# muditbhargava66/FFT-implementation-in-C

Measured on AMD Instinct MI355X. Metric: Gpoint/s + achieved HBM GB/s, batched 1D c2c FFT at 1/2/4/8 MI355X, higher is better.
Workload: dtype f32; 1 GPU; N=1048576 fp32 complex, batch=512 per GPU (BASELINE configs[2], north-star); n=1048576, batch_per_gpu=512, batch_total=512, direction=forward, placement=out-of-place, parallelism=batch index sharded over 1 GPU(s), one process per GPU, no collectives, algo=auto, passes=2, chunk_batch=128, bluestein_m=0, schedule=team kernel: one HBM round trip, a whole transform per team of CUs of one XCD, team_tiles=4, team_status=0, device=AMD Radeon Graphics (gfx950:sramecc+:xnack-, 256 CUs)

## Files before the change

fft-implementation-in-c_amd/csrc/fft_device.h:

```cpp
#pragma once

#include <stdint.h>

#if defined(FFT_EMU)
#include <cstring>
namespace emu {
struct dim3_ { unsigned x, y, z; };
extern thread_local dim3_ threadIdx_;
extern thread_local dim3_ blockIdx_;
extern dim3_ blockDim_;
extern dim3_ gridDim_;
extern thread_local unsigned char* smem_;
void sync_threads();
long long clock_ticks();
extern int xcc_skew;
unsigned shfl_xor_u32(unsigned v, int mask);
}
#define FFT_KERNEL
#define FFT_DEVICE inline
#define FFT_HOST_DEVICE inline
#define FFT_TID ((int)emu::threadIdx_.x)
#define FFT_BID ((long long)emu::blockIdx_.x)
#define FFT_NTHREADS ((int)emu::blockDim_.x)
#define FFT_NBLOCKS ((long long)emu::gridDim_.x)
// ... 9 lines not shown
    memcpy(w, &v, sizeof(T));
    for (unsigned i = 0; i < sizeof(T) / 4; i++) w[i] = shfl_xor_u32(w[i], mask);
    memcpy(&v, w, sizeof(T));
    return v;
}
}
#define FFT_SHFL_XOR(v, mask) emu::shfl_xor_any(v, mask)
#define FFT_XOR_EXCHANGE(v, mask, upper) emu::shfl_xor_any(v, mask)
#define FFT_OPAQUE(v) (void)(v)
#define FFT_LAUNCH_BOUNDS(n)
#define FFT_LAUNCH_BOUNDS2(n, w)
#define FFT_RESTRICT
#define FFT_UNROLL
#define FFT_NOUNROLL
#define FFT_UNROLL_N(n)
#include <sched.h>
#define FFT_XCC_ID(nteams) ((unsigned)((emu::blockIdx_.x + ((emu::xcc_skew && emu::blockIdx_.x == 0) ? 1u : 0u)) % (unsigned)(nteams)))
#define FFT_ATOMIC_ADD_AGENT(p, v) __atomic_fetch_add((p), (v), __ATOMIC_SEQ_CST)
#define FFT_ATOMIC_ADD_AGENT_RELAXED(p, v) __atomic_fetch_add((p), (v), __ATOMIC_SEQ_CST)
#define FFT_ATOMIC_ADD_AGENT_RELEASE(p, v) __atomic_fetch_add((p), (v), __ATOMIC_SEQ_CST)
#define FFT_FENCE_ACQUIRE_AGENT() __atomic_thread_fence(__ATOMIC_SEQ_CST)
#define FFT_ATOMIC_LOAD_AGENT(p) __atomic_load_n((p), __ATOMIC_SEQ_CST)
#define FFT_ATOMIC_STORE_AGENT(p, v) __atomic_store_n((p), (v), __ATOMIC_SEQ_CST)
namespace emu {
inline unsigned cas_u32(unsigned* p, unsigned expected, unsigned desired) {
    __atomic_compare_exchange_n(p, &expected, desired, false, __ATOMIC_SEQ_CST, __ATOMIC_SEQ_CST);
    return expected;
}
void test_delay();
bool test_drop();
}
#define FFT_ATOMIC_CAS_AGENT(p, expected, desired) emu::cas_u32((p), (expected), (desired))
#define FFT_TEST_DELAY() emu::test_delay()
#define FFT_TEST_DROP() emu::test_drop()
#define FFT_L2_FLAG_STORE(p, v) __atomic_store_n((p), (v), __ATOMIC_SEQ_CST)
#define FFT_L2_FLAG_LOAD(p) __atomic_load_n((p), __ATOMIC_SEQ_CST)
#define FFT_L2_COUNT_ADD(p) ((void)__atomic_fetch_add((p), 1u, __ATOMIC_SEQ_CST))
#define FFT_L2_COUNT_POLL(p) __atomic_load_n((p), __ATOMIC_SEQ_CST)
#define FFT_L2_COUNT_POLL2(p) ((unsigned long long)__atomic_load_n((p), __ATOMIC_SEQ_CST) | ((unsigned long long)__atomic_load_n((p) + 1, __ATOMIC_SEQ_CST) << 32))
#define FFT_L2_STORE64(p, lo, hi) __atomic_store_n((unsigned long long*)(p), (unsigned long long)(lo) | ((unsigned long long)(hi) << 32), __ATOMIC_SEQ_CST)
#define FFT_L2_LOAD64(p) __atomic_load_n((const unsigned long long*)(p), __ATOMIC_SEQ_CST)
#define FFT_PAIR_UNIT 1
#define FFT_LDS_FRESH() __atomic_thread_fence(__ATOMIC_SEQ_CST)
#define FFT_SCHED_BARRIER() ((void)0)
#define FFT_WAIT_VM0() __atomic_thread_fence(__ATOMIC_SEQ_CST)
#define FFT_SLEEP() sched_yield()
// ... 43 lines not shown
    }
    return __shfl_xor(v, mask, 64);
}
__device__ __forceinline__ double fft_xor_exchange(double v, int mask, bool) { return __shfl_xor(v, mask, 64); }
#ifdef FFT_NO_OPAQUE
#define FFT_OPAQUE(v) (void)(v)
#else
#define FFT_OPAQUE(v) asm volatile("" : "+v"(v))
#endif
#define FFT_LAUNCH_BOUNDS(n) __launch_bounds__(n)
#define FFT_LAUNCH_BOUNDS2(n, w) __launch_bounds__(n, w)
#define FFT_RESTRICT __restrict__
#define FFT_UNROLL _Pragma("unroll")
#define FFT_NOUNROLL _Pragma("nounroll")
#define FFT_PRAGMA_(x) _Pragma(#x)
#define FFT_UNROLL_N(n) FFT_PRAGMA_(unroll n)
#define FFT_XCC_ID(nteams) ((unsigned)__builtin_amdgcn_s_getreg((3 << 11) | (0 << 6) | 20) & 15u)
#define FFT_ATOMIC_ADD_AGENT(p, v) __hip_atomic_fetch_add((p), (v), __ATOMIC_ACQ_REL, __HIP_MEMORY_SCOPE_AGENT)
#define FFT_ATOMIC_ADD_AGENT_RELAXED(p, v) __hip_atomic_fetch_add((p), (v), __ATOMIC_RELAXED, __HIP_MEMORY_SCOPE_AGENT)
#define FFT_ATOMIC_ADD_AGENT_RELEASE(p, v) __hip_atomic_fetch_add((p), (v), __ATOMIC_RELEASE, __HIP_MEMORY_SCOPE_AGENT)
#define FFT_FENCE_ACQUIRE_AGENT() __builtin_amdgcn_fence(__ATOMIC_ACQUIRE, "agent")
#define FFT_ATOMIC_LOAD_AGENT(p) __hip_atomic_load((p), __ATOMIC_ACQUIRE, __HIP_MEMORY_SCOPE_AGENT)
#define FFT_ATOMIC_STORE_AGENT(p, v) __hip_atomic_store((p), (v), __ATOMIC_RELEASE, __HIP_MEMORY_SCOPE_AGENT)
__device__ __forceinline__ unsigned fft_cas_agent(unsigned* p, unsigned expected, unsigned desired) {
    __hip_atomic_compare_exchange_strong(p, &expected, desired, __ATOMIC_ACQ_REL, __ATOMIC_ACQUIRE, __HIP_MEMORY_SCOPE_AGENT);
    return expected;
}
#define FFT_ATOMIC_CAS_AGENT(p, expected, desired) fft_cas_agent((p), (expected), (desired))
#define FFT_TEST_DELAY() ((void)0)
#define FFT_TEST_DROP() false
#define FFT_L2_FLAG_STORE(p, v) asm volatile("global_store_dword %0, %1, off" ::"v"((unsigned*)(p)), "v"((unsigned)(v)) : "memory")
#define FFT_L2_FLAG_LOAD(p) __hip_atomic_load((p), __ATOMIC_RELAXED, __HIP_MEMORY_SCOPE_AGENT)
#define FFT_L2_COUNT_ADD(p) asm volatile("global_atomic_add %0, %1, off" ::"v"((unsigned*)(p)), "v"(1u) : "memory")
#define FFT_L2_COUNT_POLL(p) fft_scalar_load_glc((const unsigned*)(p))
__device__ __forceinline__ unsigned fft_scalar_load_glc(const unsigned* p) {
    unsigned v;
    asm volatile("s_load_dword %0, %1, 0x0 glc\n\ts_waitcnt lgkmcnt(0)" : "=s"(v) : "s"(p) : "memory");
    return v;
}
#define FFT_L2_COUNT_POLL2(p) fft_scalar_load2_glc((const unsigned*)(p))
__device__ __forceinline__ unsigned long long fft_scalar_load2_glc(const unsigned* p) {
    unsigned long long v;
    asm volatile("s_load_dwordx2 %0, %1, 0x0 glc\n\ts_waitcnt lgkmcnt(0)" : "=s"(v) : "s"(p) : "memory");
    return v;
}
#define FFT_L2_STORE64(p, lo, hi) fft_l2_store64((unsigned*)(p), (unsigned)(lo), (unsigned)(hi))
// ... 205 lines not shown
#endif

#if !defined(FFT_EMU)
typedef float fft_lds_v2f __attribute__((ext_vector_type(2)));
__device__ __forceinline__ cpx<float> fft_lds_ld64(const cpx<float>* p) {
    const fft_lds_v2f v = *(const volatile __attribute__((address_space(3))) fft_lds_v2f*)(const __attribute__((address_space(3))) void*)p;
    cpx<float> r;
    r.re = v.x;
    r.im = v.y;
    return r;
}
__device__ __forceinline__ void fft_lds_st64(cpx<float>* p, cpx<float> a) {
    fft_lds_v2f v = {a.re, a.im};
    *(volatile __attribute__((address_space(3))) fft_lds_v2f*)(__attribute__((address_space(3))) void*)p = v;
}
#endif

template <typename T>
struct alignas(16) vec16 {
    static constexpr int V = 16 / (int)sizeof(cpx<T>);
    cpx<T> c[V];
};

template <typename T, int V>
struct alignas(V * sizeof(cpx<T>)) lvec {
    cpx<T> c[V];
};

FFT_DEVICE unsigned bitrev32(unsigned v, int log2n) {
    v = ((v >> 1) & 0x55555555u) | ((v & 0x55555555u) << 1);
    v = ((v >> 2) & 0x33333333u) | ((v & 0x33333333u) << 2);
    v = ((v >> 4) & 0x0F0F0F0Fu) | ((v & 0x0F0F0F0Fu) << 4);
    v = ((v >> 8) & 0x00FF00FFu) | ((v & 0x00FF00FFu) << 8);
    v = (v >> 16) | (v << 16);
    return log2n > 0 ? (v >> (32 - log2n)) : 0u;
}

}
```

fft-implementation-in-c_amd/csrc/fft_engine.h:

```cpp
#pragma once

#include <math.h>
#include <stdio.h>
#include <stdlib.h>
#include <string.h>

#include <algorithm>
#include <type_traits>
#include <vector>

#include "fft_kernels.h"
#include "fft_kernels_chain.h"
#include "fft_rows_list.h"
#include "fft_team_list.h"
#include "fft_team_defer.h"
#include "fft_mixed_radix.h"
#if defined(FFT_EMU)
#include "fft_team_quad.h"
#include "fft_wide_row.h"
#else
#include "fft_team_quad_decl.h"
#define FFT_WIDE_DECL_ONLY
#include "fft_wide_row.h"
#endif
// ... 274 lines not shown
        if (d.n_teams > fftk::TEAM_CTL_MAX_TEAMS) return;
        d.data_bytes = 2 * (SZ << log2TE);
        d.tables_elems = (int)(L2 / 2 + L1 + L2);
        d.smem_bytes = d.data_bytes + d.tables_elems * SZ + 32;
        if (d.smem_bytes > rt->max_lds_bytes()) return;
        std::vector<cpx<T>> blob, part;
        make_twiddle_table<T>(blob, L1 * L2, L2 / 2, 1);
        make_twiddle_table<T>(part, L1, L1, 1);
        blob.insert(blob.end(), part.begin(), part.end());
        make_twiddle_table<T>(part, L2, L2, 1);
        blob.insert(blob.end(), part.begin(), part.end());
        make_twiddle_table<T>(part, L1 * L2, 2, L2 / 2);
        blob.push_back(part[1]);
        blob.push_back(part[0]);
        d.scratch_bytes = ((size_t)SZ << (log2TE + d.log2TS)) * 2 * (size_t)d.n_teams;
        d.tables = (cpx<T>*)rt->dmalloc(blob.size() * SZ);
        d.scratch = (unsigned char*)rt->dmalloc(d.scratch_bytes);
        d.sticky = (unsigned*)rt->dmalloc((fftk::TEAM_STICKY_WORDS + fftk::TEAM_CTL_WORDS) * sizeof(unsigned));
        d.ctl = d.sticky ? d.sticky + fftk::TEAM_STICKY_WORDS : nullptr;
        if (!d.tables || !d.scratch || !d.sticky) {
            rt->dfree(d.tables); rt->dfree(d.scratch); rt->dfree(d.sticky);
            return;
        }
        rt->memset_async(d.sticky, 0, fftk::TEAM_STICKY_WORDS * sizeof(unsigned));
        rt->h2d(d.tables, blob.data(), blob.size() * SZ);
        {
            const long long mib = d.log2TS >= 4 ? 128 : 256;
            d.min_batch = mode == 1 ? (int)std::max<long long>(2ll * d.n_teams, (mib << 20) / ((long long)SZ << log2n)) : d.n_teams;
        }
        if (rt->policy.team_min_batch > 0) d.min_batch = rt->policy.team_min_batch;
        (void)batch;
        d.ok = true;
        team = d;
    }

    void launch_team_quad(const fftk::TeamParams<T>& tp) {
        const long long grid = (long long)team.n_xcc << team.log2seats;
#define FFT_QUAD_GO(TT, E, RA, RB, L1, L2, TS, SLOTS)                                                                            \
    if constexpr (std::is_same<T, TT>::value) {                                                                                  \
        if (log2n == (L1) + (L2) && team.log2TS == (TS) && team.quad_slots == (SLOTS))                                           \
            return rt->launch_coresident(fftk::team_quad_kernel<TT, E, RA, RB, L1, L2, TS, SLOTS>, grid, team.nthreads, (size_t)team.smem_bytes, tp); \
    }
        FFT_QUAD_INSTANCES(FFT_QUAD_GO)
#undef FFT_QUAD_GO
        (void)grid;
    }

// ... 48 lines not shown
            make_twiddle_table<T>(part, L2, 1ll << d.sa2_bits, 1);
            std::copy(part.begin(), part.end(), blob.begin() + d.o_sa2);
            make_twiddle_table<T>(part, L2, 1ll << (d.log2L2 - d.sa2_bits), 1ll << d.sa2_bits);
            std::copy(part.begin(), part.end(), blob.begin() + d.o_sb2);
        }
        const long long n = 1ll << log2n;
        make_twiddle_table<T>(part, n, 1ll << d.t0_bits, 1);
        std::copy(part.begin(), part.end(), blob.begin() + d.o_t0);
        make_twiddle_table<T>(part, n, 1ll << (log2n - d.t0_bits), 1ll << d.t0_bits);
        std::copy(part.begin(), part.end(), blob.begin() + d.o_t1);
        d.defer = d.NT == 4 && !d.asplit && rt->team_defer(SZ, log2n);
        d.pair = d.defer && V == 2 && d.log2CB >= 1 && rt->team_pair(SZ, log2n);
        d.nodefer = d.pair && rt->team_nodefer(SZ, log2n);
        d.alll2 = d.nodefer && rt->team_alll2(SZ, log2n);
        d.scratch_bytes = ((size_t)SZ << (log2TE + d.log2TS)) * (d.defer ? 4 : 2) * (size_t)d.n_teams;
        d.tables = (cpx<T>*)rt->dmalloc(blob.size() * SZ);
        d.scratch = (unsigned char*)rt->dmalloc(d.scratch_bytes);
        d.sticky = (unsigned*)rt->dmalloc((fftk::TEAM_STICKY_WORDS + fftk::TEAM_CTL_WORDS) * sizeof(unsigned));
        d.ctl = d.sticky ? d.sticky + fftk::TEAM_STICKY_WORDS : nullptr;
        if (!d.tables || !d.scratch || !d.sticky) {
            rt->dfree(d.tables); rt->dfree(d.scratch); rt->dfree(d.sticky);
            return;
        }
        rt->memset_async(d.sticky, 0, fftk::TEAM_STICKY_WORDS * sizeof(unsigned));
        rt->h2d(d.tables, blob.data(), blob.size() * SZ);
        {
            long long mib = 512;
            if (SZ == 8) mib = d.log2TS >= 5 ? 256 : d.log2TS == 4 ? 512 : d.log2TS == 3 ? 1024 : d.log2TS == 2 ? 4096 : 2048;
            d.min_batch = mode == 1 ? (int)std::max<long long>(4ll * d.n_teams, (mib << 20) / ((long long)SZ << log2n)) : d.n_teams;
        }
        if (rt->policy.team_min_batch > 0) d.min_batch = rt->policy.team_min_batch;
        (void)batch;
        d.ok = true;
        team = d;
    }

    template <int GEO, bool ASPLIT, bool PAIR>
    void launch_team_geo(const fftk::TeamParams<T>& tp) {
        const long long grid = (long long)team.n_xcc << team.log2seats;
        if (team.defer && team.pair && team.nodefer && team.alll2 && PAIR)
            rt->launch_coresident(fftk::team_defer_kernel<T, 8 * V, GEO, PAIR, PAIR, PAIR>, grid, team.nthreads, (size_t)team.smem_bytes, tp);
        else if (team.defer && team.pair && team.nodefer && PAIR)
            rt->launch_coresident(fftk::team_defer_kernel<T, 8 * V, GEO, PAIR, PAIR>, grid, team.nthreads, (size_t)team.smem_bytes, tp);
        else if (team.defer && team.pair && PAIR)
            rt->launch_coresident(fftk::team_defer_kernel<T, 8 * V, GEO, PAIR>, grid, team.nthreads, (size_t)team.smem_bytes, tp);
        else if (team.defer)
            rt->launch_coresident(fftk::team_defer_kernel<T, 8 * V, GEO>, grid, team.nthreads, (size_t)team.smem_bytes, tp);
// ... 56 lines not shown
        tp.timeout_ticks = rt->team_timeout_ticks();
        tp.form_timeout_ticks = (team_fallbacks > 0 || team_suspensions > 0) ? std::max<long long>(1, rt->team_form_timeout_ticks() / 10) : rt->team_form_timeout_ticks();
        tp.sticky = team.sticky;
        static const int ablate = FFT_EXP_ENV("FFT_HIP_TEAM_ABLATE") ? atoi(FFT_EXP_ENV("FFT_HIP_TEAM_ABLATE")) : 0;
        tp.ablate = ablate;
        static const int dma_split = FFT_EXP_ENV("FFT_HIP_TEAM_DMA_SPLIT") ? atoi(FFT_EXP_ENV("FFT_HIP_TEAM_DMA_SPLIT")) : 4;
        tp.dma_split = dma_split;
        static const int dma_split2 = FFT_EXP_ENV("FFT_HIP_TEAM_DMA_SPLIT2") ? atoi(FFT_EXP_ENV("FFT_HIP_TEAM_DMA_SPLIT2")) : 8;
        tp.dma_split2 = dma_split2;
        static const int seat_rot = FFT_EXP_ENV("FFT_HIP_TEAM_SEAT_ROT") ? atoi(FFT_EXP_ENV("FFT_HIP_TEAM_SEAT_ROT")) : 0;
        tp.seat_rot = seat_rot;
        const int dynamic = FFT_EXP_ENV("FFT_HIP_TEAM_DYNAMIC") ? atoi(FFT_EXP_ENV("FFT_HIP_TEAM_DYNAMIC")) : 1;
        tp.dynamic = team.quad ? dynamic : 0;
        static const int tile_rot = FFT_EXP_ENV("FFT_HIP_TEAM_TILE_ROT") ? atoi(FFT_EXP_ENV("FFT_HIP_TEAM_TILE_ROT")) : -1;
        tp.tile_rot = tile_rot >= 0 ? tile_rot : (team.pair ? 2 : 4);
        static const int nt_mask = FFT_EXP_ENV("FFT_HIP_TEAM_NT") ? atoi(FFT_EXP_ENV("FFT_HIP_TEAM_NT")) : -1;
        tp.nt_mask = nt_mask >= 0 ? nt_mask : (team.quad ? 7 : team.nodefer ? 7 : team.pair ? 3 : 1);
        static const int tune = FFT_EXP_ENV("FFT_HIP_TEAM_TUNE") ? atoi(FFT_EXP_ENV("FFT_HIP_TEAM_TUNE")) : 0;
        tp.tune = tune;
        tp.force_no_teams = team_force_fallback ? 1 : 0;
        tp.trace = team.trace;
        tp.trace_events = team.trace_events;
        tp.scale = scale;
        rt->memset_async(team.ctl, 0, fftk::TEAM_CTL_WORDS * sizeof(unsigned));
        if (team.quad) {
            launch_team_quad(tp);
            return;
        }
#if defined(FFT_EMU)
        switch (team.NT) {
            case 1: launch_team_emu<1>(tp); break;
            case 2: launch_team_emu<2>(tp); break;
            default: launch_team_emu<4>(tp); break;
        }
#else
#define FFT_TEAM_ROW(TT, LOG2N, GEO, ASPLIT, PAIR)               \
    if constexpr (std::is_same<T, TT>::value) {                  \
        if (log2n == (LOG2N)) return launch_team_geo<GEO, ASPLIT, PAIR>(tp); \
    }
        FFT_TEAM_INSTANCES(FFT_TEAM_ROW)
#undef FFT_TEAM_ROW
#endif
    }

    static int layout_tables(PassDesc& p) {
        const long long L = 1ll << p.log2L;
        p.sa_bits = (L * SZ > 8192) ? (p.log2L + 1) / 2 : p.log2L;
// ... 752 lines not shown
        const size_t last = passes.size() - 1;
        for (int b0 = 0; b0 < nb; b0 += chunk) {
            const int cb = (nb - b0) < chunk ? (nb - b0) : chunk;
            const cpx<T>* src = in + (size_t)b0 * (size_t)ip;
            cpx<T>* dst = out + (size_t)b0 * (size_t)op;
            launch_pass_hooked(0, src, scratch, cb, inverse, (T)1, h, 1, 0);
            rt->mark(0);
            if (passes.size() == 3) {
                launch_pass(1, scratch, scratch, cb, inverse, (T)1);
                rt->mark(1);
            }
            launch_pass_hooked(last, scratch, dst, cb, inverse, scale, h, 2, (long long)b0 * h.post_tab_b);
            rt->mark((int)last);
        }
    }

    static long long grid_for(long long total, int block) {
        long long g = (total + block - 1) / block;
        if (g > 16384) g = 16384;
        if (g < 1) g = 1;
        return g;
    }

    int recover_after_timeout(bool timed_out) {
        int lost = 0;
        if (timed_out) {
            team.ok = false;
            team_disabled = true;
            std::vector<TeamExec> log;
            log.swap(team_log);
            const size_t nbytes = (size_t)SZ << log2n;
            auto overlap = [&](const void* a, size_t abytes, const void* b, size_t bbytes) {
                const char *pa = (const char*)a, *pb = (const char*)b;
                return pa < pb + bbytes && pb < pa + abytes;
            };
            std::vector<char> bad(log.size(), 0);
            for (size_t k = 0; k < log.size(); k++) {
                const TeamExec& e = log[k];
                const size_t bytes = nbytes * (size_t)e.nb;
                bool ok = team_replay && team_log_dropped == 0 && !overlap(e.in, bytes, e.out, bytes);
                for (size_t j = 0; ok && j < log.size(); j++) {
                    if (j == k) continue;
                    const size_t jb = nbytes * (size_t)log[j].nb;
                    if (!overlap(e.in, bytes, log[j].out, jb)) continue;
                    if (j > k || bad[j]) ok = false;
                }
                if (ok && e.staged && (k + 1 < log.size())) {
                    for (size_t j = k + 1; ok && j < log.size(); j++)
                        if (log[j].staged && overlap(e.in, bytes, log[j].in, nbytes * (size_t)log[j].nb)) ok = false;
                }
                if (!ok) { bad[k] = 1; lost++; continue; }
// ... 461 lines not shown
```

fft-implementation-in-c_amd/csrc/fft_hip_backend.hip:

```cpp
#include <hip/hip_runtime.h>
#include <pthread.h>
#include <stdio.h>
#include <stdlib.h>
#include <string.h>

#include <map>
#include <new>
#include <set>
#include <tuple>
#include <type_traits>
#include <utility>
#include <vector>

#include "../../include/fft_hip.h"
#include "fft_kernels.h"
#include "fft_rows_list.h"

namespace fftk {
#define FFT_EXTERN(T, E, FAM) \
    extern template __global__ void tile_fft_kernel<T, E, 1, FAM, LOAD_LCONTIG, STORE_LCONTIG, false, 0>(TileParams<T>);
FFT_ROWS_LIST(FFT_EXTERN)
#undef FFT_EXTERN
#define FFT_EXTERN_FIXED(T, LOG2L, LOG2C) \
    extern template __global__ void tile_fft_kernel<T, 4, 1, FAM_R4, LOAD_LCONTIG, STORE_LCONTIG, false, ((LOG2L) << 8) | (LOG2C)>(TileParams<T>);
// ... 285 lines not shown
    if (!core->team.ctl || !core->team.sticky) return -1;
    unsigned st = 0, sticky[2] = {0, 0};
    if (hipMemcpy(&st, core->team.ctl + fftk::TEAM_CTL_STATUS, sizeof(st), hipMemcpyDeviceToHost) != hipSuccess ||
        hipMemcpy(sticky, core->team.sticky, sizeof(sticky), hipMemcpyDeviceToHost) != hipSuccess) {
        (void)hipGetLastError();
        return -1;
    }
    const int launches = core->team_pending;
    core->team_pending = 0;
    if (sticky[fftk::TEAM_STICKY_TIMEOUTS]) st = fftk::TEAM_STATUS_TIMEOUT;
    if (sticky[0] || sticky[1]) (void)hipMemset(core->team.sticky, 0, sizeof(sticky));
    core->team_last_status = (int)st;
    if (st == fftk::TEAM_STATUS_TIMEOUT) {
        const int lost = core->recover_after_timeout(true);
        if (hipStreamSynchronize(core->rt->stream) != hipSuccess) (void)hipGetLastError();
        if (lost)
            fprintf(stderr, "fft_hip: a team kernel barrier timed out; %d execute(s) since the last sync could not be repeated (their input "
                            "is gone, overwritten by a later execute, or not the caller's to keep) and hold invalid data; this plan continues "
                            "with the multi-pass schedule\n", lost);
        else
            fprintf(stderr, "fft_hip: a team kernel barrier timed out; the executes since the last sync were repeated on the multi-pass "
                            "schedule, which this plan keeps from now on\n");
        if (!lost) st = fftk::TEAM_STATUS_NO_TEAMS;
        core->team_last_status = (int)st;
    } else if ((int)sticky[fftk::TEAM_STICKY_FALLBACKS] >= launches && launches > 0) {
        core->team_fallbacks += launches;
        if (core->team_fallbacks >= 3) {
            core->team_suspend = 64 << (core->team_suspensions < 4 ? core->team_suspensions : 4);
            core->team_suspensions++;
            core->team_fallbacks = 0;
            fprintf(stderr, "fft_hip: the team kernel could not form its XCD teams three times in a row; this plan runs its next %d "
                            "executes on the multi-pass schedule before it tries again\n", core->team_suspend);
        }
    } else {
        core->team_fallbacks = 0;
        if (st == fftk::TEAM_STATUS_OK && launches > 0) {
            core->team_seen_ok();
            core->team_suspensions = 0;
        }
    }
    if (st != fftk::TEAM_STATUS_TIMEOUT) {
        core->team_log.clear();
        core->team_log_dropped = 0;
        core->team_stage_used = 0;
    }
    return (int)st;
}
// ... 1116 lines not shown
```

fft-implementation-in-c_amd/csrc/fft_team.h:

```cpp
#pragma once

#include "fft_kernels.h"

#ifndef FFT_TEAM_DMA_FIRST
#define FFT_TEAM_DMA_FIRST(nch) ((nch) / 2)
#endif

namespace fftk {

enum {
    TEAM_CTL_REGISTERED = 0,
    TEAM_CTL_NEXT = 2,
    TEAM_CTL_STATUS = 1,
    TEAM_CTL_COUNT = 32,
    TEAM_CTL_FLAGS = 32 + 32 * 16,
    TEAM_CTL_MAX_TEAMS = 256,
    TEAM_CTL_PAIR = 32 + 32 * 16 + 32 * TEAM_CTL_MAX_TEAMS,
    TEAM_CTL_WORDS = TEAM_CTL_PAIR + 32 * 3 * TEAM_CTL_MAX_TEAMS
};
enum { TEAM_STICKY_TIMEOUTS = 0, TEAM_STICKY_FALLBACKS = 1, TEAM_STICKY_WORDS = 32 };
enum { TEAM_STATUS_OK = 0, TEAM_STATUS_NO_TEAMS = 1, TEAM_STATUS_TIMEOUT = 2 };
constexpr unsigned TEAM_CTL_POISON = 0x80000000u;

template <typename T>
struct TeamParams {
    const cpx<T>* in;
    cpx<T>* out;
    const cpx<T>* tables;
    unsigned char* scratch;
    unsigned* ctl;
    unsigned* sticky;
    int tables_bytes;
    int data_bytes;
    int log2L1, log2L2, log2CA, log2CB, log2TS;
    int n_xcc;
    int log2seats;
// ... 56 lines not shown
        }
        FFT_SLEEP();
    }
    FFT_FENCE_ACQUIRE_AGENT();
    unsigned xcc_rank = 0;
    if (ok) {
        unsigned cnts[16];
        FFT_UNROLL
        for (int x = 0; x < 16; x++) cnts[x] = FFT_L2_FLAG_LOAD(&p.ctl[TEAM_CTL_COUNT + 32 * x]);
        int full = 0;
        FFT_UNROLL
        for (int x = 0; x < 16; x++) {
            const unsigned cnt = cnts[x];
            if (cnt == (1u << p.log2seats)) {
                full++;
                if ((unsigned)x < xcc) xcc_rank++;
            } else if (cnt != 0u) {
                ok = 0;
            }
        }
        if (full != p.n_xcc) ok = 0;
    }
    if (p.force_no_teams) ok = 0;
    if (!ok && FFT_ATOMIC_CAS_AGENT(&p.ctl[TEAM_CTL_STATUS], 0u, (unsigned)TEAM_STATUS_NO_TEAMS) == 0u)
        FFT_ATOMIC_ADD_AGENT(&p.sticky[TEAM_STICKY_FALLBACKS], 1u);
    sh[0] = slot;
    sh[1] = xcc_rank;
    sh[2] = ok;
    sh[3] = 0;
}

template <typename T>
FFT_DEVICE void team_report_timeout(const TeamParams<T>& p) {
    FFT_ATOMIC_CAS_AGENT(&p.ctl[TEAM_CTL_STATUS], 0u, (unsigned)TEAM_STATUS_TIMEOUT);
    FFT_ATOMIC_ADD_AGENT(&p.sticky[TEAM_STICKY_TIMEOUTS], 1u);
}

#ifndef FFT_TEAM_TW_TREE
#define FFT_TEAM_TW_TREE 1
#endif
#ifndef FFT_TEAM_TW_TREE_F64
#define FFT_TEAM_TW_TREE_F64 1
#endif
#ifndef FFT_TEAM_TW_TREE_F64_MIN
#define FFT_TEAM_TW_TREE_F64_MIN 17
#endif

#define FFT_TEAM_GEO(l1, l2, ca, cb, ts) ((l1) | ((l2) << 5) | ((ca) << 10) | ((cb) << 15) | ((ts) << 20))

template <class Hook>
struct StageHookAt {
    Hook& hook;
    int s, total;
    FFT_DEVICE void operator()() const { hook(s, total); }
};

template <typename T, int GEO>
struct TeamTwTree {
// ... 182 lines not shown
    unsigned char* const work = smem + tile_bytes;
    unsigned char* const tab_bytes = smem + 2 * tile_bytes;
    const unsigned land_lds = FFT_LDS_ADDR(land);
    {
        const vec16<T>* src = reinterpret_cast<const vec16<T>*>(p.tables);
        vec16<T>* dst = reinterpret_cast<vec16<T>*>(tab_bytes);
        for (int i = tid_invariant; i < (p.tables_bytes >> 4); i += nthreads) dst[i] = src[i];
    }
    const cpx<T>* tab = reinterpret_cast<const cpx<T>*>(tab_bytes);
    unsigned* const sh = reinterpret_cast<unsigned*>(tab_bytes + p.tables_bytes);
    StageTw<T> twA, twB;
    twA.sa = tab;
    twA.sb = tab + p.o_sb1;
    twA.sa_bits = team_stage_table_bits(SZ, ASPLIT ? log2L1 - 1 : log2L1);
    twA.log2L = ASPLIT ? log2L1 - 1 : log2L1;
    twB.sa = tab + p.o_sa2;
    twB.sb = tab + p.o_sb2;
    twB.sa_bits = team_stage_table_bits(SZ, log2L2);
    twB.log2L = log2L2;

    if (tid_invariant == 0) team_form(p, sh);
    FFT_SYNC();
    FFT_LDS_FRESH();
    if (!sh[2]) return;
    const unsigned seat = (FFT_UNIFORM(sh[0]) + (unsigned)p.seat_rot) & ((1u << p.log2seats) - 1u);
    const int c = (int)(seat & (unsigned)(TS - 1));
    const int team = (int)((FFT_UNIFORM(sh[1]) << (p.log2seats - log2TS)) + (seat >> log2TS));
    const int n_teams = p.n_xcc << (p.log2seats - log2TS);

    unsigned char* const sbase = p.scratch + (size_t)team * 2 * phase_bytes;
    unsigned* const flags = p.ctl + TEAM_CTL_FLAGS + 32 * team;

    int n_ev = 0;
    auto ev = [&]() __attribute__((always_inline)) {
        if (p.trace && tid_invariant == 0 && n_ev < p.trace_events - 1) {
            p.trace[(long long)FFT_BID * p.trace_events + n_ev] = FFT_CLOCK();
            n_ev++;
        }
    };
    ev();
    if (p.trace && tid_invariant == 0 && p.trace_events > 1) p.trace[(long long)FFT_BID * p.trace_events + p.trace_events - 1] = (team << 8) | c;

    constexpr bool COUNTER = (NT == 4);
    auto wait_all = [&](unsigned g) __attribute__((always_inline)) {
        FFT_LDS_FRESH();
        if (sh[3]) return;
        if (tid_invariant < FFT_TEAM_POLL_LANES) {
// ... 278 lines not shown
                } else if (p.nt_mask & 2) {
                    FFT_UNROLL
                    for (int q = 0; q < E / 2; q++) FFT_STORE16_NT(dst0 + q * dstep, v[q]);
                } else {
                    FFT_UNROLL
                    for (int q = 0; q < E / 2; q++) dst0[q * dstep] = v[q];
                }
            } else {
                FFT_UNROLL
                for (int e = 0; e < E; e++) {
                    const long long K = rB + (e << log2TPCB);
                    *reinterpret_cast<cpx<T>*>(outb + (K << log2L1) + k1 + jB) = x[0][e][0];
                }
            }
            ev();
            if (ph + 1 < NT) {
                FFT_WAIT_VM_LE(NCH);
                FFT_SYNC_LDS();
                arrive(g0 + ph + 2);
                ev();
            }
        }
    }
}

}
```

fft-implementation-in-c_amd/csrc/fft_team_defer.h:

```cpp
#pragma once

#include "fft_team.h"

namespace fftk {

#ifndef FFT_TEAM_INPLACE
#define FFT_TEAM_INPLACE 0
#endif
template <typename T, int E, int GEO, bool PAIR = false, bool NODEFER = false, bool ALLL2 = false>
FFT_KERNEL void FFT_LAUNCH_BOUNDS2(4096 * vec16<T>::V / E, 16 * vec16<T>::V / E) team_defer_kernel(TeamParams<T> p) {
    constexpr int NT = 4;
    constexpr bool TREE = TeamTwTree<T, GEO>::value;
    static_assert(!PAIR || vec16<T>::V == 2, "paired result stores: fp32 only");
    static_assert(!ALLL2 || (NODEFER && PAIR), "ALLL2 is a variant of the paired NODEFER schedule");
    constexpr int V16 = vec16<T>::V;
    constexpr int log2V16 = Log2<V16>::value;
    constexpr int log2E = Log2<E>::value;
    constexpr int NCH = E / V16;
    constexpr int SZ = (int)sizeof(cpx<T>);
    constexpr int EP = E / NT;
    constexpr int NK = 2;
    constexpr int log2NT = 2;
    constexpr int NRS_EVEN = PAIR ? 0 : NCH, NRS_ODD = PAIR ? 2 * NCH : NCH;
    FFT_DYN_SMEM(smem);
// ... 23 lines not shown
    auto dma_img = [&]() __attribute__((always_inline)) -> unsigned char* { return INPL ? (par ? buf0 : buf1) : buf0; };
    auto dma_lds = [&]() __attribute__((always_inline)) -> unsigned { return INPL ? (par ? buf0_lds : buf0_lds + tile_bytes) : buf0_lds; };
    auto tile_done = [&]() __attribute__((always_inline)) { if (INPL) par ^= 1; };
    {
        const vec16<T>* src = reinterpret_cast<const vec16<T>*>(p.tables);
        vec16<T>* dst = reinterpret_cast<vec16<T>*>(tab_bytes);
        for (int i = tid_invariant; i < (p.tables_bytes >> 4); i += nthreads) dst[i] = src[i];
    }
    const cpx<T>* tab = reinterpret_cast<const cpx<T>*>(tab_bytes);
    unsigned* const sh = reinterpret_cast<unsigned*>(tab_bytes + p.tables_bytes);
    StageTw<T> twA, twB;
    twA.sa = tab;
    twA.sb = tab + p.o_sb1;
    twA.sa_bits = team_stage_table_bits(SZ, log2L1);
    twA.log2L = log2L1;
    twB.sa = tab + p.o_sa2;
    twB.sb = tab + p.o_sb2;
    twB.sa_bits = team_stage_table_bits(SZ, log2L2);
    twB.log2L = log2L2;

    if (tid_invariant == 0) team_form(p, sh);
    FFT_SYNC();
    FFT_LDS_FRESH();
    if (!sh[2]) return;
    const unsigned seat = (FFT_UNIFORM(sh[0]) + (unsigned)p.seat_rot) & ((1u << p.log2seats) - 1u);
    const int c = (int)(seat & (unsigned)(TS - 1));
    const int team = (int)((FFT_UNIFORM(sh[1]) << (p.log2seats - log2TS)) + (seat >> log2TS));
    const int n_teams = p.n_xcc << (p.log2seats - log2TS);
    const int M = team < p.nb ? (p.nb - team + n_teams - 1) / n_teams : 0;
    if (M == 0) return;
    if (FFT_TEST_DROP()) return;

    unsigned char* const sbase = p.scratch + (size_t)team * 4 * phase_bytes;
    unsigned* const flags = p.ctl + TEAM_CTL_FLAGS + 32 * team;

    int n_ev = 0;
    auto ev = [&]() __attribute__((always_inline)) {
        if (p.trace && tid_invariant == 0 && n_ev < p.trace_events - 1) {
            p.trace[(long long)FFT_BID * p.trace_events + n_ev] = FFT_CLOCK();
            n_ev++;
        }
    };
    ev();
    if (p.trace && tid_invariant == 0 && p.trace_events > 1) p.trace[(long long)FFT_BID * p.trace_events + p.trace_events - 1] = (team << 8) | c;

    auto wait_all = [&](int g) __attribute__((always_inline)) {
        FFT_LDS_FRESH();
        if (g <= 0 || sh[3]) return;
        if (tid_invariant < FFT_TEAM_POLL_LANES) {
            const long long t0 = FFT_CLOCK();
            while ((int)(FFT_L2_COUNT_POLL(flags) - ((unsigned)g << log2TS)) < 0) {
                if (FFT_CLOCK() - t0 > p.timeout_ticks) {
                    team_report_timeout(p);
                    sh[3] = 1;
// ... 305 lines not shown
            if (s > 1) return;
            if (it + 1 < M && !NODEFER) {
                dma_column_tile(in_of(it + 1), 0, slot_i0(s), slot_i1(s, total));
            } else {
                if (s == 0) wait_all(G + 4);
                dma_row_tile(NODEFER ? S1 : S2, slot_i0(s), slot_i1(s, total));
            }
        });
        if constexpr (NODEFER) {
            FFT_WAIT_VM_LE(NRS_EVEN);
            FFT_SYNC_LDS();
            arrive(G + 5);
            row_body(outb, 3, [&](int s, int total) {
                if (s > 1) return;
                if (it + 1 < M) dma_column_tile(in_of(it + 1), 0, slot_i0(s), slot_i1(s, total));
            });
        }
    }
    if constexpr (!NODEFER) {
        FFT_WAIT_VM0();
        FFT_SYNC_LDS();
        row_body(out_of(M - 1), 3, [&](int, int) {});
    }
}

}
```

fft-implementation-in-c_amd/csrc/fft_team_quad.h:

```cpp
#pragma once

#include "fft_team_quad_decl.h"

#ifndef QUAD_LDS_SINGLE
#define QUAD_LDS_SINGLE 1
#endif
#if QUAD_LDS_SINGLE
#define QUAD_LD(p) FFT_LDS_LD64(p)
#define QUAD_ST(p, v) FFT_LDS_ST64((p), (v))
#else
#define QUAD_LD(p) (*(p))
#define QUAD_ST(p, v) (*(p) = (v))
#endif
namespace fftk {
template <typename T>
FFT_DEVICE cpx<T> quad_ld(const cpx<T>* p) {
    if constexpr (sizeof(T) == 4) return QUAD_LD(p);
    else return *p;
}
template <typename T>
FFT_DEVICE void quad_st(cpx<T>* p, cpx<T> v) {
    if constexpr (sizeof(T) == 4) QUAD_ST(p, v);
    else *p = v;
}
// ... 163 lines not shown
    const long long t_entry = p.trace ? FFT_CLOCK() : 0;

    const int tid0 = FFT_TID;
    const int tid = tid0;
    auto img_b = [&](int i) __attribute__((always_inline)) -> unsigned char* { return smem + (size_t)i * IMG; };
    unsigned char* const tab_bytes = smem + 2 * (size_t)IMG;
    const unsigned img_lds0 = FFT_LDS_ADDR(smem);
    {
        const vec16<T>* src = reinterpret_cast<const vec16<T>*>(p.tables);
        vec16<T>* dst = reinterpret_cast<vec16<T>*>(tab_bytes);
        for (int i = tid; i < (p.tables_bytes >> 4); i += NTHR) dst[i] = src[i];
    }
    const cpx<T>* const t0 = reinterpret_cast<const cpx<T>*>(tab_bytes);
    const cpx<T>* const wlA = t0 + L2 / 2;
    const cpx<T>* const wlB = wlA + L1;
    unsigned* const sh = reinterpret_cast<unsigned*>(tab_bytes + p.tables_bytes);

    if (tid == 0) {
        sh[4] = 0;
        team_form(p, sh);
    }
    FFT_SYNC();
    FFT_LDS_FRESH();
    if (!sh[2]) return;
    const unsigned seat = (FFT_UNIFORM(sh[0]) + (unsigned)p.seat_rot) & ((1u << p.log2seats) - 1u);
    const int s = (int)(seat & (unsigned)(TS - 1));
    const int team = (int)((FFT_UNIFORM(sh[1]) << (p.log2seats - LOG2TS)) + (seat >> LOG2TS));
    const int n_teams = p.n_xcc << (p.log2seats - LOG2TS);
    if (team >= p.nb) return;
    if (FFT_TEST_DROP()) return;

    unsigned char* const sbase = p.scratch + (size_t)team * (PAIR ? 1 : SLOTS) * SLOT;
    const size_t slot_stride = FFT_ABLATE(p.ablate & 32) ? 0 : FFT_ABLATE(p.ablate & 16) ? SLOT / 2 : SLOT;
    unsigned* const flags = p.ctl + TEAM_CTL_FLAGS + 32 * team;

    int n_ev = 0;
    auto ev = [&]() __attribute__((always_inline)) {
        if (p.trace && tid == 0 && n_ev < p.trace_events - 2) {
            p.trace[(long long)FFT_BID * p.trace_events + n_ev] = FFT_CLOCK();
            n_ev++;
        }
    };
    ev();
    if (p.trace && tid == 0 && p.trace_events > 1) p.trace[(long long)FFT_BID * p.trace_events + p.trace_events - 1] = (team << 8) | s;
    if (p.trace && tid == 0 && p.trace_events > 2) p.trace[(long long)FFT_BID * p.trace_events + p.trace_events - 2] = t_entry;

    auto wait_all = [&](int g, bool learn = false) __attribute__((always_inline)) {
        FFT_LDS_FRESH();
        if (sh[3]) return;
        if (FFT_ABLATE(p.ablate & 8)) {
            FFT_SYNC_LDS();
            return;
        }
// ... 539 lines not shown
            else {
                FFT_UNROLL
                for (int k = 0; k < E; k++) zt[r][k] = v[k];
            }
        }
        }
        ev();
        if (DEFER) {
            out_prev = outb;
        } else {
            FFT_UNROLL
            for (int a = 0; a < 4; a++) final_part(a, outb);
        }
        ev();
        cur = nxt;
    }
    if (DEFER && out_prev) {
        FFT_LDS_FRESH();
        if (!sh[3]) {
            FFT_UNROLL
            for (int a = 0; a < 4; a++) final_part(a, out_prev);
        }
    }
}

}
```

Before: 220.6 Gpoint/s.

## Reset team control block in-kernel on exit instead of host memset per launch

Removes the per-execute memset of the team control words before each team-kernel launch. Instead, the last block of each XCC clears its team flags (and pair lines), and the last exiting block resets the global control words and writes the final status. The control block is zeroed once at plan creation, and again on host recovery after a timeout. This saves a memset launch and its stream serialization per execute, at the cost of extra exit atomics and stores in the kernel tail and more complex reset logic.

```diff
diff --git a/fft-implementation-in-c_amd/csrc/fft_device.h b/fft-implementation-in-c_amd/csrc/fft_device.h
--- a/fft-implementation-in-c_amd/csrc/fft_device.h
+++ b/fft-implementation-in-c_amd/csrc/fft_device.h
@@ -55,6 +55,7 @@
 #define FFT_FENCE_ACQUIRE_AGENT() __atomic_thread_fence(__ATOMIC_SEQ_CST)
 #define FFT_ATOMIC_LOAD_AGENT(p) __atomic_load_n((p), __ATOMIC_SEQ_CST)
 #define FFT_ATOMIC_STORE_AGENT(p, v) __atomic_store_n((p), (v), __ATOMIC_SEQ_CST)
+#define FFT_STORE_AGENT_RELAXED(p, v) __atomic_store_n((p), (v), __ATOMIC_SEQ_CST)
 namespace emu {
 inline unsigned cas_u32(unsigned* p, unsigned expected, unsigned desired) {
     __atomic_compare_exchange_n(p, &expected, desired, false, __ATOMIC_SEQ_CST, __ATOMIC_SEQ_CST);
@@ -144,6 +145,7 @@
 #define FFT_FENCE_ACQUIRE_AGENT() __builtin_amdgcn_fence(__ATOMIC_ACQUIRE, "agent")
 #define FFT_ATOMIC_LOAD_AGENT(p) __hip_atomic_load((p), __ATOMIC_ACQUIRE, __HIP_MEMORY_SCOPE_AGENT)
 #define FFT_ATOMIC_STORE_AGENT(p, v) __hip_atomic_store((p), (v), __ATOMIC_RELEASE, __HIP_MEMORY_SCOPE_AGENT)
+#define FFT_STORE_AGENT_RELAXED(p, v) __hip_atomic_store((p), (v), __ATOMIC_RELAXED, __HIP_MEMORY_SCOPE_AGENT)
 __device__ __forceinline__ unsigned fft_cas_agent(unsigned* p, unsigned expected, unsigned desired) {
     __hip_atomic_compare_exchange_strong(p, &expected, desired, __ATOMIC_ACQ_REL, __ATOMIC_ACQUIRE, __HIP_MEMORY_SCOPE_AGENT);
     return expected;
@@ -395,6 +397,10 @@
     cpx<T> c[V];
 };
 
+struct alignas(16) uint4_words {
+    unsigned w[4];
+};
+
 template <typename T, int V>
 struct alignas(V * sizeof(cpx<T>)) lvec {
     cpx<T> c[V];
diff --git a/fft-implementation-in-c_amd/csrc/fft_engine.h b/fft-implementation-in-c_amd/csrc/fft_engine.h
--- a/fft-implementation-in-c_amd/csrc/fft_engine.h
+++ b/fft-implementation-in-c_amd/csrc/fft_engine.h
@@ -320,7 +320,7 @@
             rt->dfree(d.tables); rt->dfree(d.scratch); rt->dfree(d.sticky);
             return;
         }
-        rt->memset_async(d.sticky, 0, fftk::TEAM_STICKY_WORDS * sizeof(unsigned));
+        rt->memset_async(d.sticky, 0, (fftk::TEAM_STICKY_WORDS + fftk::TEAM_CTL_WORDS) * sizeof(unsigned));
         rt->h2d(d.tables, blob.data(), blob.size() * SZ);
         {
             const long long mib = d.log2TS >= 4 ? 128 : 256;
@@ -415,7 +415,7 @@
             rt->dfree(d.tables); rt->dfree(d.scratch); rt->dfree(d.sticky);
             return;
         }
-        rt->memset_async(d.sticky, 0, fftk::TEAM_STICKY_WORDS * sizeof(unsigned));
+        rt->memset_async(d.sticky, 0, (fftk::TEAM_STICKY_WORDS + fftk::TEAM_CTL_WORDS) * sizeof(unsigned));
         rt->h2d(d.tables, blob.data(), blob.size() * SZ);
         {
             long long mib = 512;
@@ -518,7 +518,6 @@
         tp.trace = team.trace;
         tp.trace_events = team.trace_events;
         tp.scale = scale;
-        rt->memset_async(team.ctl, 0, fftk::TEAM_CTL_WORDS * sizeof(unsigned));
         if (team.quad) {
             launch_team_quad(tp);
             return;
@@ -1317,11 +1316,17 @@
         return g;
     }
 
+    void zero_team_ctl() {
+        if (!team.ctl) return;
+        rt->memset_async(team.ctl, 0, fftk::TEAM_CTL_STATUS * sizeof(unsigned));
+        rt->memset_async(team.ctl + fftk::TEAM_CTL_STATUS + 1, 0, (fftk::TEAM_CTL_WORDS - fftk::TEAM_CTL_STATUS - 1) * sizeof(unsigned));
+    }
     int recover_after_timeout(bool timed_out) {
         int lost = 0;
         if (timed_out) {
             team.ok = false;
             team_disabled = true;
+            zero_team_ctl();
             std::vector<TeamExec> log;
             log.swap(team_log);
             const size_t nbytes = (size_t)SZ << log2n;
diff --git a/fft-implementation-in-c_amd/csrc/fft_hip_backend.hip b/fft-implementation-in-c_amd/csrc/fft_hip_backend.hip
--- a/fft-implementation-in-c_amd/csrc/fft_hip_backend.hip
+++ b/fft-implementation-in-c_amd/csrc/fft_hip_backend.hip
@@ -331,7 +331,7 @@
             fprintf(stderr, "fft_hip: a team kernel barrier timed out; the executes since the last sync were repeated on the multi-pass "
                             "schedule, which this plan keeps from now on\n");
         if (!lost) st = fftk::TEAM_STATUS_NO_TEAMS;
-        core->team_last_status = (int)st;
+        core->team_last_status = lost ? -1 : (int)st;
     } else if ((int)sticky[fftk::TEAM_STICKY_FALLBACKS] >= launches && launches > 0) {
         core->team_fallbacks += launches;
         if (core->team_fallbacks >= 3) {
diff --git a/fft-implementation-in-c_amd/csrc/fft_team.h b/fft-implementation-in-c_amd/csrc/fft_team.h
--- a/fft-implementation-in-c_amd/csrc/fft_team.h
+++ b/fft-implementation-in-c_amd/csrc/fft_team.h
@@ -12,6 +12,9 @@
     TEAM_CTL_REGISTERED = 0,
     TEAM_CTL_NEXT = 2,
     TEAM_CTL_STATUS = 1,
+    TEAM_CTL_EXIT = 3,
+    TEAM_CTL_TIMED_OUT = 4,
+    TEAM_CTL_GLOBAL_WORDS = 32 + 32 * 16,
     TEAM_CTL_COUNT = 32,
     TEAM_CTL_FLAGS = 32 + 32 * 16,
     TEAM_CTL_MAX_TEAMS = 256,
@@ -114,8 +117,6 @@
         if (full != p.n_xcc) ok = 0;
     }
     if (p.force_no_teams) ok = 0;
-    if (!ok && FFT_ATOMIC_CAS_AGENT(&p.ctl[TEAM_CTL_STATUS], 0u, (unsigned)TEAM_STATUS_NO_TEAMS) == 0u)
-        FFT_ATOMIC_ADD_AGENT(&p.sticky[TEAM_STICKY_FALLBACKS], 1u);
     sh[0] = slot;
     sh[1] = xcc_rank;
     sh[2] = ok;
@@ -124,8 +125,52 @@
 
 template <typename T>
 FFT_DEVICE void team_report_timeout(const TeamParams<T>& p) {
-    FFT_ATOMIC_CAS_AGENT(&p.ctl[TEAM_CTL_STATUS], 0u, (unsigned)TEAM_STATUS_TIMEOUT);
+    FFT_ATOMIC_ADD_AGENT(&p.ctl[TEAM_CTL_TIMED_OUT], 1u);
     FFT_ATOMIC_ADD_AGENT(&p.sticky[TEAM_STICKY_TIMEOUTS], 1u);
+}
+
+template <typename T>
+FFT_DEVICE void team_leave(const TeamParams<T>& p, unsigned* sh, int log2TS, bool pair) {
+    const int tid = FFT_TID, nthreads = FFT_NTHREADS;
+    FFT_WAIT_VM0();
+    FFT_SYNC();
+    FFT_LDS_FRESH();
+    const unsigned formed = sh[2];
+    if (tid == 0) {
+        unsigned last = 0;
+        if (formed) {
+            const unsigned xcc = FFT_XCC_ID(p.n_xcc);
+            if (FFT_ATOMIC_ADD_AGENT_RELAXED(&p.ctl[TEAM_CTL_COUNT + 32 * xcc + 1], 1u) + 1u == (1u << p.log2seats)) last |= 1u;
+        }
+        sh[0] = last;
+    }
+    FFT_SYNC();
+    FFT_LDS_FRESH();
+    if (sh[0] & 1u) {
+        const unsigned tpx = 1u << (p.log2seats - log2TS), first = sh[1] * tpx;
+        uint4_words* const f = reinterpret_cast<uint4_words*>(p.ctl + TEAM_CTL_FLAGS + 32 * first);
+        for (unsigned i = (unsigned)tid; i < 8u * tpx; i += (unsigned)nthreads) f[i] = uint4_words{0u, 0u, 0u, 0u};
+        if (pair) {
+            const unsigned lines = 2u * (1u << log2TS) + 1u;
+            uint4_words* const q = reinterpret_cast<uint4_words*>(p.ctl + TEAM_CTL_PAIR + 32 * lines * first);
+            for (unsigned i = (unsigned)tid; i < 8u * lines * tpx; i += (unsigned)nthreads) q[i] = uint4_words{0u, 0u, 0u, 0u};
+        }
+    }
+    if (formed && !(sh[0] & 1u)) return;
+    FFT_SYNC();
+    if (tid == 0) {
+        const unsigned tickets = formed ? (unsigned)p.n_xcc : (unsigned)FFT_NBLOCKS;
+        sh[0] = FFT_ATOMIC_ADD_AGENT_RELAXED(&p.ctl[TEAM_CTL_EXIT], 1u) + 1u == tickets ? 2u : 0u;
+    }
+    FFT_SYNC();
+    FFT_LDS_FRESH();
+    if (!(sh[0] & 2u)) return;
+    FFT_FENCE_ACQUIRE_AGENT();
+    unsigned status = TEAM_STATUS_NO_TEAMS;
+    if (formed) status = FFT_L2_FLAG_LOAD(&p.ctl[TEAM_CTL_TIMED_OUT]) ? (unsigned)TEAM_STATUS_TIMEOUT : (unsigned)TEAM_STATUS_OK;
+    else if (tid == 0) FFT_ATOMIC_ADD_AGENT(&p.sticky[TEAM_STICKY_FALLBACKS], 1u);
+    FFT_SYNC();
+    for (int i = tid; i < TEAM_CTL_GLOBAL_WORDS; i += nthreads) FFT_STORE_AGENT_RELAXED(&p.ctl[i], i == TEAM_CTL_STATUS ? status : 0u);
 }
 
 #ifndef FFT_TEAM_TW_TREE
@@ -354,7 +399,7 @@
     if (tid_invariant == 0) team_form(p, sh);
     FFT_SYNC();
     FFT_LDS_FRESH();
-    if (!sh[2]) return;
+    if (!sh[2]) return team_leave(p, sh, log2TS, false);
     const unsigned seat = (FFT_UNIFORM(sh[0]) + (unsigned)p.seat_rot) & ((1u << p.log2seats) - 1u);
     const int c = (int)(seat & (unsigned)(TS - 1));
     const int team = (int)((FFT_UNIFORM(sh[1]) << (p.log2seats - log2TS)) + (seat >> log2TS));
@@ -679,6 +724,7 @@
             }
         }
     }
-}
-
-}
+    team_leave(p, sh, log2TS, false);
+}
+
+}
diff --git a/fft-implementation-in-c_amd/csrc/fft_team_defer.h b/fft-implementation-in-c_amd/csrc/fft_team_defer.h
--- a/fft-implementation-in-c_amd/csrc/fft_team_defer.h
+++ b/fft-implementation-in-c_amd/csrc/fft_team_defer.h
@@ -69,14 +69,14 @@
     if (tid_invariant == 0) team_form(p, sh);
     FFT_SYNC();
     FFT_LDS_FRESH();
-    if (!sh[2]) return;
+    if (!sh[2]) return team_leave(p, sh, log2TS, false);
     const unsigned seat = (FFT_UNIFORM(sh[0]) + (unsigned)p.seat_rot) & ((1u << p.log2seats) - 1u);
     const int c = (int)(seat & (unsigned)(TS - 1));
     const int team = (int)((FFT_UNIFORM(sh[1]) << (p.log2seats - log2TS)) + (seat >> log2TS));
     const int n_teams = p.n_xcc << (p.log2seats - log2TS);
     const int M = team < p.nb ? (p.nb - team + n_teams - 1) / n_teams : 0;
-    if (M == 0) return;
-    if (FFT_TEST_DROP()) return;
+    if (M == 0) return team_leave(p, sh, log2TS, false);
+    if (FFT_TEST_DROP()) return team_leave(p, sh, log2TS, false);
 
     unsigned char* const sbase = p.scratch + (size_t)team * 4 * phase_bytes;
     unsigned* const flags = p.ctl + TEAM_CTL_FLAGS + 32 * team;
@@ -428,6 +428,7 @@
         FFT_SYNC_LDS();
         row_body(out_of(M - 1), 3, [&](int, int) {});
     }
+    team_leave(p, sh, log2TS, false);
 }
 
 }
diff --git a/fft-implementation-in-c_amd/csrc/fft_team_quad.h b/fft-implementation-in-c_amd/csrc/fft_team_quad.h
--- a/fft-implementation-in-c_amd/csrc/fft_team_quad.h
+++ b/fft-implementation-in-c_amd/csrc/fft_team_quad.h
@@ -209,13 +209,13 @@
     }
     FFT_SYNC();
     FFT_LDS_FRESH();
-    if (!sh[2]) return;
+    if (!sh[2]) return team_leave(p, sh, LOG2TS, PAIR);
     const unsigned seat = (FFT_UNIFORM(sh[0]) + (unsigned)p.seat_rot) & ((1u << p.log2seats) - 1u);
     const int s = (int)(seat & (unsigned)(TS - 1));
     const int team = (int)((FFT_UNIFORM(sh[1]) << (p.log2seats - LOG2TS)) + (seat >> LOG2TS));
     const int n_teams = p.n_xcc << (p.log2seats - LOG2TS);
-    if (team >= p.nb) return;
-    if (FFT_TEST_DROP()) return;
+    if (team >= p.nb) return team_leave(p, sh, LOG2TS, PAIR);
+    if (FFT_TEST_DROP()) return team_leave(p, sh, LOG2TS, PAIR);
 
     unsigned char* const sbase = p.scratch + (size_t)team * (PAIR ? 1 : SLOTS) * SLOT;
     const size_t slot_stride = FFT_ABLATE(p.ablate & 32) ? 0 : FFT_ABLATE(p.ablate & 16) ? SLOT / 2 : SLOT;
@@ -801,6 +801,7 @@
             for (int a = 0; a < 4; a++) final_part(a, out_prev);
         }
     }
-}
-
-}
+    team_leave(p, sh, LOG2TS, PAIR);
+}
+
+}
```

Measured after the change: 219.4 Gpoint/s. No clear change (-0.5%).
